# PRBonn/OverlapNet

Hardware: NVIDIA H100
Metric: scan-pairs/sec (overlap+yaw) at 64x900 (higher is better)
Workload: dtype f16

## Files before the change

### overlapnet_b200/csrc/network_tc.cu

```cuda
#include "common.cuh"
#include "hopper.cuh"

#include <cuda_fp16.h>
#include <stddef.h>
#include <stdlib.h>

namespace ovn {

using namespace hopper;

constexpr int WF = 360;
constexpr int CF = 128;
constexpr int S15 = 15;
constexpr int NB = 24;
constexpr int PAIR_ROWS = NB * NB;
constexpr int K4_PITCH = CF;

struct TcState {
  Buffer<__half> w1p;
  Buffer<__half> w2p;
  Buffer<__half> w3p;
  Buffer<float> b2eff;
  Buffer<__half> wres[kMaxLegLayers];
  Buffer<__half> actp[2];
// ... 313 lines not shown
#pragma unroll
            for (int j = 0; j < 8; ++j) sto[tt][h][j] = st + ((j ^ (ib & 7)) << 4);
          }
      }
      const uint32_t wb = S.right.slot(ui);
      PIPE_WAIT(S.right.wait(ui), kErrDeltaRightConsumer);
      float acc[2][32];
#pragma unroll
      for (int j = 0; j < 8; ++j) {
        const float m0 = __half2float(__float2half_rn(-__ldg(mu_o1 + j * 8 + 2 * t)));
        const float m1 = __half2float(__float2half_rn(-__ldg(mu_o1 + j * 8 + 2 * t + 1)));
#pragma unroll
        for (int tt = 0; tt < 2; ++tt) {
          acc[tt][4 * j + 0] = m0; acc[tt][4 * j + 1] = m1;
          acc[tt][4 * j + 2] = m0; acc[tt][4 * j + 3] = m1;
        }
      }
      uint32_t Lr[2][2][4];
#pragma unroll 1
      for (int grp = 0; grp < K4_NGROUPS; ++grp, ++gi) {
        const int cc = grp / K4_CHUNK_GROUPS, dj0 = (grp - K4_CHUNK_GROUPS * cc) * K4_GROUP;
        if (dj0 == 0) {
#pragma unroll
          for (int tt = 0; tt < 2; ++tt)
#pragma unroll
            for (int h = 0; h < 2; ++h) {
              const int r = rows[tt][h] < blk.rows ? rows[tt][h] : blk.rows - 1;
              const uint4 v = *reinterpret_cast<const uint4*>(S.L + r * K4_PITCH + ((cc ^ (r & 1)) << 5) + 8 * t);
              Lr[tt][h][0] = v.x; Lr[tt][h][1] = v.y; Lr[tt][h][2] = v.z; Lr[tt][h][3] = v.w;
            }
        }
        const uint32_t s = S.w1.slot(gi);
        const uint64_t bdesc = desc_kmajor(b_base + s * (K4_GROUP * K4_BSLICE), 1024, 128, kNoSwizzle);
        const int par = (jb + dj0) & 1;
        const __half* rw = S.Rw[wb] + dj0 * K4_PITCH + 8 * t;
        const __half* rp[2] = {rw + ((cc ^ par) << 5), rw + ((cc ^ par ^ 1) << 5)};
        uint4 rv = *reinterpret_cast<const uint4*>(rp[0]);
        PIPE_WAIT(S.w1.wait(gi), kErrDeltaW1Consumer);
        uint32_t A[2][2][4];
#pragma unroll
        for (int sl = 0; sl < K4_GROUP; ++sl)
#pragma unroll
          for (int kk = 0; kk < 2; ++kk) {
            const uint32_t r0 = kk ? rv.z : rv.x, r1 = kk ? rv.w : rv.y;
#pragma unroll
            for (int tt = 0; tt < 2; ++tt) {
              A[tt][kk][0] = absdiff_h2(Lr[tt][0][2 * kk], r0);
              A[tt][kk][1] = absdiff_h2(Lr[tt][1][2 * kk], r0);
              A[tt][kk][2] = absdiff_h2(Lr[tt][0][2 * kk + 1], r1);
              A[tt][kk][3] = absdiff_h2(Lr[tt][1][2 * kk + 1], r1);
            }
            wgmma_fence();
#pragma unroll
            for (int tt = 0; tt < 2; ++tt)
              wgmma_m64n64k16_rs(acc[tt], A[tt][kk], bdesc + ((sl * K4_BSLICE + kk * 2048) >> 4));
            wgmma_commit();
            if (kk == 1 && sl + 1 < K4_GROUP) rv = *reinterpret_cast<const uint4*>(rp[(sl + 1) & 1] + (sl + 1) * K4_PITCH);
            wgmma_wait<1>();
          }
        wgmma_wait<0>();
        S.w1.release(gi);
      }
      S.right.release(ui);
      if (jb == NB - 1 || u == u_end - 1) S.left.release(pi - 1);
      if (!S.o1s.wait_free(ui)) { atomicExch(err, kErrDeltaO1Consumer); goto done; }
#pragma unroll
      for (int tt = 0; tt < 2; ++tt)
#pragma unroll
        for (int h = 0; h < 2; ++h) {
          if (rows[tt][h] >= blk.rows) continue;
#pragma unroll
          for (int j = 0; j < 8; ++j)
            *reinterpret_cast<uint32_t*>(smem_raw + sto[tt][h][j]) = pack_h2(acc[tt][4 * j + 2 * h], acc[tt][4 * j + 2 * h + 1]);
        }
      fence_proxy_async_smem();
      S.o1s.publish(ui);
    }
  }
done:
  return;
}

constexpr int TC_WG = 2;
constexpr int TC_THREADS = TC_WG * 128 + 32;
constexpr int TC_ROWS = TC_WG * 128;
constexpr uint32_t C2_TILE = 128 * 64 * 2;
constexpr int C2_RING = 3;

struct C2Smem {
  __half A[C2_RING][TC_WG][C2_TILE / 2];
  __half B[C2_RING][2][C2_TILE / 2];
  MbarRing<C2_RING> ring;
};
constexpr size_t C2_SMEM = sizeof(C2Smem) + 1024;
static_assert(C2_SMEM <= 232448, "k_conv2_wgmma shared memory");
static_assert(offsetof(C2Smem, B) % 1024 == 0 && C2_TILE % 1024 == 0, "SWIZZLE_128B tiles on 1024-byte boundaries");

__global__ void __launch_bounds__(TC_THREADS, 1)
k_conv2_wgmma(const __half* __restrict__ o1, const __half* __restrict__ W2s, const float* __restrict__ bias2,
              const float* __restrict__ mu_x3, __half* __restrict__ x3, int64_t out_pitch, int64_t M, int fault,
              int* __restrict__ err) {
  if (fault) {
    if (threadIdx.x == 0 && blockIdx.x == 0) atomicExch(err, kErrInjectedFault);
    return;
  }
  extern __shared__ __align__(128) uint8_t smem_raw[];
  C2Smem& S = *reinterpret_cast<C2Smem*>(smem_raw + ((1024 - (smem_u32(smem_raw) & 1023)) & 1023));
  const int tid = threadIdx.x, warp = tid >> 5, lane = tid & 31;
  const Share tiles = work_share((M + TC_ROWS - 1) / TC_ROWS, blockIdx.x, gridDim.x);
  if (tid == 0) {
    S.ring.init(TC_WG * 4);
    mbar_fence_init();
  }
  __syncthreads();

  if (warp == TC_WG * 4) {
    if (lane == 0) {
      uint32_t gi = 0;
      for (int64_t tile = tiles.begin; tile < tiles.end; ++tile)
        for (int di = 0; di < S15; ++di, ++gi) {
          const uint32_t s = S.ring.slot(gi);
          PIPE_WAIT(S.ring.acquire(gi, 4 * C2_TILE), kErrConv2Producer);
          for (int h = 0; h < TC_WG; ++h)
            bulk_g2s(S.A[s][h], o1 + ((size_t)(tile * TC_WG + h) * S15 + di) * (C2_TILE / 2), C2_TILE, S.ring.bar(gi));
          bulk_g2s(S.B[s], W2s + (size_t)di * C2_TILE, 2 * C2_TILE, S.ring.bar(gi));
        }
    }
  } else {
    const int wg = warp >> 2, wi = warp & 3, g = lane >> 2, t = lane & 3;
    uint32_t gi = 0;
    bool failed = false;
    for (int64_t tile = tiles.begin; tile < tiles.end; ++tile) {
      float acc[2][64];
#pragma unroll
      for (int sub = 0; sub < 2; ++sub)
#pragma unroll
        for (int e = 0; e < 64; ++e) acc[sub][e] = 0.f;
#pragma unroll 1
      for (int di = 0; di < S15; ++di, ++gi) {
        const uint32_t s = S.ring.slot(gi);
        INFLIGHT_WAIT(S.ring.wait(gi), kErrConv2Consumer);
        const uint32_t a_base = smem_u32(S.A[s][wg]), b_base = smem_u32(S.B[s][0]);
        wgmma_fence();
#pragma unroll
        for (int kk = 0; kk < 4; ++kk)
#pragma unroll
          for (int part = 0; part < 2; ++part) {
            const uint64_t bd = desc_kmajor(b_base + part * C2_TILE + kk * 32, 16, 1024, kSwizzle128B);
#pragma unroll
            for (int sub = 0; sub < 2; ++sub)
              wgmma_m64n128k16_ss(acc[sub], desc_kmajor(a_base + sub * (C2_TILE / 2) + kk * 32, 16, 1024, kSwizzle128B), bd);
          }
        wgmma_commit();
        wgmma_wait<1>();
        if (di > 0) S.ring.release(gi - 1);
      }
      wgmma_wait<0>();
      if (failed) goto done;
      S.ring.release(gi - 1);
#pragma unroll
      for (int sub = 0; sub < 2; ++sub)
#pragma unroll
        for (int h = 0; h < 2; ++h) {
          const int64_t m = tile * TC_ROWS + wg * 128 + sub * 64 + wi * 16 + g + 8 * h;
          if (m >= M) continue;
#pragma unroll
          for (int j = 0; j < 16; ++j) {
            const int n = j * 8 + 2 * t;
            const float a = fmaxf(acc[sub][4 * j + 2 * h] + __ldg(bias2 + n), 0.f) - __ldg(mu_x3 + n);
            const float b = fmaxf(acc[sub][4 * j + 2 * h + 1] + __ldg(bias2 + n + 1), 0.f) - __ldg(mu_x3 + n + 1);
            *reinterpret_cast<uint32_t*>(x3 + ((size_t)j * out_pitch + m) * 8 + 2 * t) = pack_h2(a, b);
          }
        }
    }
  }
done:
  return;
}

constexpr int C3_AROWS = TC_ROWS + 2 * NB + 2;
constexpr uint32_t C3_PLANE = C3_AROWS * 16;
constexpr uint32_t C3_SLAB = 4 * 128 * 16;
constexpr int C3_GROUP = 2;
constexpr int C3_NSTAGES = 36 / C3_GROUP;
constexpr int C3_RING = 4;

struct C3Smem {
  __half A[2][16 * C3_PLANE / 2];
  __half B[C3_RING][C3_GROUP * C3_SLAB / 2];
  MbarRing<C3_RING> w3;
  MbarRing<2> x3;
};
static_assert(sizeof(C3Smem) <= 232448, "k_conv3_wgmma shared memory");
static_assert(offsetof(C3Smem, B) % 16 == 0 && C3_PLANE % 16 == 0, "bulk-copy alignment");

__global__ void __launch_bounds__(TC_THREADS, 1)
k_conv3_wgmma(const __half* __restrict__ X3, int64_t a_pitch, const __half* __restrict__ W3p, const float* __restrict__ bias,
              int64_t M, const float* __restrict__ wd, float* __restrict__ partial, int* __restrict__ err) {
  extern __shared__ __align__(128) uint8_t smem_raw[];
  C3Smem& S = *reinterpret_cast<C3Smem*>(smem_raw);
  const int tid = threadIdx.x, warp = tid >> 5, lane = tid & 31;
  const Share tiles = work_share(2 * ((M + TC_ROWS - 1) / TC_ROWS), blockIdx.x, gridDim.x);
  if (tid == 0) {
    S.w3.init(TC_WG * 4);
    S.x3.init(TC_WG * 4);
    mbar_fence_init();
  }
  __syncthreads();

  if (warp == TC_WG * 4) {
    if (lane == 0) {
      const uint32_t nt = (uint32_t)(tiles.end - tiles.begin);
      uint32_t ai = 0, gi = 0;
      for (uint32_t ti = 0; ti < nt; ++ti) {
        const int nh = (int)((tiles.begin + ti) & 1);
        for (int st = 0; st < C3_NSTAGES; ++st, ++gi) {
          while (ai < nt && ai <= ti + 1) {
            if (ai > ti) {
              if (!S.x3.try_acquire(ai, 16 * C3_PLANE)) break;
            } else {
              PIPE_WAIT(S.x3.acquire(ai, 16 * C3_PLANE), kErrConv3X3Producer);
            }
            const int64_t r0 = ((tiles.begin + ai) >> 1) * TC_ROWS;
            for (int pl = 0; pl < 16; ++pl)
              bulk_g2s(S.A[S.x3.slot(ai)] + pl * (C3_PLANE / 2), X3 + ((size_t)pl * a_pitch + r0) * 8, C3_PLANE, S.x3.bar(ai));
            ++ai;
          }
          PIPE_WAIT(S.w3.acquire(gi, C3_GROUP * C3_SLAB), kErrConv3W3Producer);
          bulk_g2s(S.B[S.w3.slot(gi)], W3p + ((size_t)nh * 36 + st * C3_GROUP) * (C3_SLAB / 2), C3_GROUP * C3_SLAB,
                   S.w3.bar(gi));
        }
      }
    }
  } else {
    const int wg = warp >> 2, wi = warp & 3, g = lane >> 2, t = lane & 3;
    const uint32_t b_base = smem_u32(S.B[0]);
    uint32_t gi = 0;
    bool failed = false;
    for (int64_t tile = tiles.begin; tile < tiles.end; ++tile) {
      const uint32_t ti = (uint32_t)(tile - tiles.begin);
      const int nh = (int)(tile & 1);
      const int64_t r0 = (tile >> 1) * TC_ROWS;
      PIPE_WAIT(S.x3.wait(ti), kErrConv3X3Consumer);
      const uint32_t a_rows = smem_u32(S.A[S.x3.slot(ti)]) + wg * 128 * 16;
      float acc[2][64];
#pragma unroll
      for (int sub = 0; sub < 2; ++sub)
#pragma unroll
        for (int e = 0; e < 64; ++e) acc[sub][e] = 0.f;
#pragma unroll 1
      for (int st = 0; st < C3_NSTAGES; ++st, ++gi) {
        const uint32_t s = S.w3.slot(gi);
        INFLIGHT_WAIT(S.w3.wait(gi), kErrConv3W3Consumer);
        wgmma_fence();
#pragma unroll
        for (int sl = 0; sl < C3_GROUP; ++sl) {
          const int slab = st * C3_GROUP + sl, tap = slab >> 2, c32 = slab & 3;
          const uint32_t a_tap = a_rows + ((tap / 3) * NB + tap % 3) * 16;
          const uint32_t slab_addr = b_base + s * (C3_GROUP * C3_SLAB) + sl * C3_SLAB;
#pragma unroll
          for (int kk = 0; kk < 2; ++kk) {
            const int c16 = c32 * 2 + kk;
            const uint64_t bd = desc_kmajor(slab_addr + kk * 4096, 2048, 128, kNoSwizzle);
#pragma unroll
            for (int sub = 0; sub < 2; ++sub)
              wgmma_m64n128k16_ss(acc[sub], desc_kmajor(a_tap + 2 * c16 * C3_PLANE + sub * 64 * 16, C3_PLANE, 128, kNoSwizzle), bd);
          }
        }
        wgmma_commit();
        wgmma_wait<1>();
        if (st > 0) S.w3.release(gi - 1);
      }
      wgmma_wait<0>();
      if (failed) goto done;
      S.w3.release(gi - 1);
      S.x3.release(ti);
#pragma unroll
      for (int sub = 0; sub < 2; ++sub)
#pragma unroll
        for (int h = 0; h < 2; ++h) {
          const int64_t r = r0 + wg * 128 + sub * 64 + wi * 16 + g + 8 * h;
          const int rem = (int)(r % PAIR_ROWS);
          const int yy = rem / NB, xx = rem - yy * NB;
          const bool valid = (r < M) && (yy < NB - 2) && (xx < NB - 2);
          const float* wrow = wd + (size_t)(valid ? (xx * (NB - 2) + yy) : 0) * 256 + nh * 128;
          float sum = 0.f;
#pragma unroll
          for (int j = 0; j < 16; ++j) {
            const int n = j * 8 + 2 * t;
            sum = fmaf(fmaxf(acc[sub][4 * j + 2 * h] + __ldg(bias + nh * 128 + n), 0.f), __ldg(wrow + n), sum);
            sum = fmaf(fmaxf(acc[sub][4 * j + 2 * h + 1] + __ldg(bias + nh * 128 + n + 1), 0.f), __ldg(wrow + n + 1), sum);
          }
          sum += __shfl_xor_sync(0xffffffffu, sum, 1);
          sum += __shfl_xor_sync(0xffffffffu, sum, 2);
          if (t == 0 && r < M) partial[r * 2 + nh] = valid ? sum : 0.f;
        }
    }
  }
done:
  return;
}

constexpr int C6_PARTS = C6_LT * C6_RT;
constexpr int C6_WG = 2;
constexpr int C6_THREADS = C6_WG * 128 + 32;
constexpr int C6_RING = 3;
constexpr int C6_GPITCH = 132;

struct C6Smem {
  __half R[C6_R_BYTES / 2];
  __half L[C6_RING][C6_L_BYTES / 2];
  float G[C6_WG][C6_LROWS * C6_GPITCH];
  MbarRing<C6_RING> left;
  MbarRing<1> right;
};
static_assert(sizeof(C6Smem) <= 232448, "k_corr_wgmma shared memory");
static_assert(offsetof(C6Smem, L) % 16 == 0, "bulk-copy alignment");

__global__ void __launch_bounds__(C6_THREADS, 1)
k_corr_wgmma(const __half* __restrict__ Lc, const int32_t* __restrict__ l_idx, const __half* __restrict__ Rc,
             int r_per_pair, int n_pairs, float* __restrict__ corr_part, int* __restrict__ err) {
  extern __shared__ __align__(128) uint8_t smem_raw[];
  C6Smem& S = *reinterpret_cast<C6Smem*>(smem_raw);
  const int tid = threadIdx.x, warp = tid >> 5, lane = tid & 31;
  const int q = blockIdx.x % C6_RT;
  const Share share = work_share((int64_t)n_pairs * C6_LT, blockIdx.x / C6_RT, gridDim.x / C6_RT);
  const int u_begin = (int)share.begin, u_end = (int)share.end;
  if (tid == 0) {
    S.left.init(4);
    S.right.init(C6_WG * 4);
    mbar_fence_init();
  }
  __syncthreads();

  if (warp == C6_WG * 4) {
    if (lane == 0) {
      uint32_t ri = 0, ui = 0;
      int key = -1;
      for (int u = u_begin; u < u_end; ++u, ++ui) {
        const int p = u / C6_LT, a = u - p * C6_LT;
        if ((r_per_pair ? p : 0) != key) {
          key = r_per_pair ? p : 0;
          PIPE_WAIT(S.right.acquire(ri, C6_R_BYTES), kErrCorrRightProducer);
          bulk_g2s(S.R, Rc + ((size_t)key * C6_RT + q) * (C6_R_BYTES / 2), C6_R_BYTES, S.right.bar(ri));
          ++ri;
        }
        PIPE_WAIT(S.left.acquire(ui, C6_L_BYTES), kErrCorrLeftProducer);
        bulk_g2s(S.L[S.left.slot(ui)], Lc + ((size_t)(l_idx ? l_idx[p] : p) * C6_LT + a) * (C6_L_BYTES / 2), C6_L_BYTES,
                 S.left.bar(ui));
      }
    }
  } else {
    const int wg = warp >> 2, wi = warp & 3, g = lane >> 2, t = lane & 3, tw = tid & 127;
    float* Gw = S.G[wg];
    const uint32_t r_base = smem_u32(S.R);
    uint32_t ri = 0, ui = 0;
    int key = -1;
    bool failed = false;
    for (int u = u_begin; u < u_end; ++u, ++ui) {
      const int p = u / C6_LT, a = u - p * C6_LT;
      if ((r_per_pair ? p : 0) != key) {
        if (key >= 0) S.right.release(ri - 1);
        key = r_per_pair ? p : 0;
        INFLIGHT_WAIT(S.right.wait(ri), kErrCorrRightConsumer);
        ++ri;
      }
      if ((int)(ui & 1) != wg) continue;
      const uint32_t s = S.left.slot(ui);
      INFLIGHT_WAIT(S.left.wait(ui), kErrCorrLeftConsumer);
      const uint32_t l_base = smem_u32(S.L[s]);
      float acc[64];
#pragma unroll
      for (int e = 0; e < 64; ++e) acc[e] = 0.f;
      wgmma_fence();
#pragma unroll
      for (int c16 = 0; c16 < 8; ++c16) {
        const uint64_t ah = desc_kmajor(l_base + c16 * 2 * C6_LROWS * 16, C6_LROWS * 16, 128, kNoSwizzle);
        const uint64_t al = desc_kmajor(l_base + C6_L_BYTES / 2 + c16 * 2 * C6_LROWS * 16, C6_LROWS * 16, 128, kNoSwizzle);
        const uint64_t bh = desc_kmajor(r_base + c16 * 2 * C6_RROWS * 16, C6_RROWS * 16, 128, kNoSwizzle);
        const uint64_t bl = desc_kmajor(r_base + C6_R_BYTES / 2 + c16 * 2 * C6_RROWS * 16, C6_RROWS * 16, 128, kNoSwizzle);
        wgmma_m64n128k16_ss(acc, ah, bh);
        wgmma_m64n128k16_ss(acc, al, bh);
        wgmma_m64n128k16_ss(acc, ah, bl);
      }
      wgmma_commit();
      wgmma_wait<0>();
      S.left.release(ui);
      named_bar_sync(1 + wg, 128);
#pragma unroll
      for (int j = 0; j < 16; ++j) {
        float* r0 = Gw + (wi * 16 + g) * C6_GPITCH + j * 8 + 2 * t;
        *reinterpret_cast<float2*>(r0) = make_float2(acc[4 * j], acc[4 * j + 1]);
        *reinterpret_cast<float2*>(r0 + 8 * C6_GPITCH) = make_float2(acc[4 * j + 2], acc[4 * j + 3]);
      }
      named_bar_sync(1 + wg, 128);
      const int i_lim = min(C6_LROWS, WF - a * C6_LROWS), j_lim = min(C6_RROWS, WF - q * C6_RROWS);
      float* out = corr_part + ((size_t)p * C6_PARTS + a * C6_RT + q) * WF;
      for (int d = tw; d < WF; d += 128) {
        const int dd = d - (C6_RROWS - 1);
        float sum = 0.f;
        if (d < C6_LROWS + C6_RROWS - 1) {
#pragma unroll 8
          for (int ii = 0; ii < C6_LROWS; ++ii) {
            const int jj = ii - dd;
            if (ii < i_lim && jj >= 0 && jj < j_lim) sum += Gw[ii * C6_GPITCH + jj];
          }
        }
        int k = (a * C6_LROWS - q * C6_RROWS + dd - WF / 2) % WF;
        if (k < 0) k += WF;
        out[k] = sum;
      }
    }
  }
done:
  return;
}

template <int EPI>
__global__ void __launch_bounds__(MMA_THREADS)
k_leg_mma(LegArgs g) {
  const int warp = threadIdx.x >> 5, lane = threadIdx.x & 31, gq = lane >> 2, t = lane & 3;
  const int64_t px0 = (int64_t)blockIdx.y * MMA_ROWS + warp * 16;
  if (px0 >= g.M) return;
  const int nz = (g.n_valid + 63) / 64;
  const int y = blockIdx.x, z = blockIdx.z % nz, slice = blockIdx.z / nz;
  const int64_t in_base = (int64_t)(y / g.runs_per_img) * g.in_img_planes + (int64_t)(y % g.runs_per_img) * g.in_run_planes;
  const int64_t pa = px0 + gq < g.M ? px0 + gq : g.M - 1, pb = px0 + gq + 8 < g.M ? px0 + gq + 8 : g.M - 1;
  const int n_slabs = g.kh * g.kw * 3;
  const size_t plane = (size_t)g.a_pitch * 8;
  const int per_tap = g.c8in / 2, n_it = g.kh * g.kw * per_tap;
  const int it0 = n_it * slice / g.n_split, it1 = n_it * (slice + 1) / g.n_split;
  float acc[8][4] = {};
#pragma unroll 1
  for (int it = it0; it < it1;) {
    const int tap = it / per_tap, dh = tap / g.kw, dw = tap - dh * g.kw;
    const int c8_end = (tap + 1) * per_tap < it1 ? g.c8in : (it1 - tap * per_tap) * 2;
    {
      const __half* Ah = g.A + (size_t)(in_base + (int64_t)dh * 2 * g.c8in) * plane + (size_t)dw * 8 + 2 * t;
      const __half* Al = Ah + (size_t)g.c8in * plane;
      const __half* Bh = g.Bp + ((size_t)(z * n_slabs + (dh * g.kw + dw) * 3) * g.c8in * 64 + gq) * 8 + 2 * t;
      const __half* Bl = Bh + (size_t)2 * g.c8in * 64 * 8;
#pragma unroll 1
      for (int c8 = (it - tap * per_tap) * 2; c8 < c8_end; c8 += 2) {
        const size_t o0 = (size_t)c8 * plane, o1 = o0 + plane;
        const uint32_t h0 = ld_h2(Ah + o0 + pa * 8), h1 = ld_h2(Ah + o0 + pb * 8), h2 = ld_h2(Ah + o1 + pa * 8), h3 = ld_h2(Ah + o1 + pb * 8);
        const uint32_t l0 = ld_h2(Al + o0 + pa * 8), l1 = ld_h2(Al + o0 + pb * 8), l2 = ld_h2(Al + o1 + pa * 8), l3 = ld_h2(Al + o1 + pb * 8);
        const size_t bo = (size_t)c8 * 64 * 8;
#pragma unroll
        for (int j = 0; j < 8; ++j) {
          const uint32_t wh0 = ld_h2(Bh + bo + j * 64), wh1 = ld_h2(Bh + bo + 64 * 8 + j * 64);
          const uint32_t wl0 = ld_h2(Bl + bo + j * 64), wl1 = ld_h2(Bl + bo + 64 * 8 + j * 64);
          mma16816(acc[j], h0, h1, h2, h3, wh0, wh1);
          mma16816(acc[j], l0, l1, l2, l3, wh0, wh1);
          mma16816(acc[j], h0, h1, h2, h3, wl0, wl1);
        }
      }
    }
    it = tap * per_tap + c8_end / 2;
  }
#pragma unroll
  for (int h = 0; h < 2; ++h) {
    const int64_t px = px0 + gq + 8 * h;
    if (px >= g.M) continue;
#pragma unroll
    for (int j = 0; j < 8; ++j) {
      const int n = z * 64 + j * 8 + 2 * t;
      if (n >= g.n_valid) continue;
      if (EPI == 5) {
        *reinterpret_cast<float2*>(g.part + (((size_t)slice * gridDim.x + y) * g.M + px) * g.n_valid + n) =
            make_float2(acc[j][2 * h], acc[j][2 * h + 1]);
        continue;
      }
      const float pre_a = acc[j][2 * h] + __ldg(g.bias + n), pre_b = acc[j][2 * h + 1] + __ldg(g.bias + n + 1);
      const float a = fmaxf(pre_a, 0.f), b = fmaxf(pre_b, 0.f);
      if (EPI == 4) {
        if (leg_act_unstorable(pre_a) || leg_act_unstorable(pre_b)) atomicCAS(g.err, 0, kErrNonFiniteOperand);
        const __half2 hi = __floats2half2_rn(a, b);
        const float2 hf = __half22float2(hi);
        const int64_t pl = (int64_t)y * g.out_run_planes + (n >> 3);
        *reinterpret_cast<__half2*>(g.out_planes + ((size_t)pl * g.out_pitch + px) * 8 + (n & 7)) = hi;
        *reinterpret_cast<uint32_t*>(g.out_planes + ((size_t)(pl + g.out_run_planes / 2) * g.out_pitch + px) * 8 + (n & 7)) =
            pack_h2(a - hf.x, b - hf.y);
      } else {
        *reinterpret_cast<float2*>(g.out_f32 + ((size_t)y * g.M + px) * g.n_valid + n) = make_float2(a, b);
      }
    }
  }
}

template <int EPI>
__global__ void __launch_bounds__(256)
k_leg_splitk_reduce(LegArgs g, int rows) {
  const int c8n = g.n_valid / 8;
  const int64_t i = (int64_t)blockIdx.x * blockDim.x + threadIdx.x;
  if (i >= (int64_t)rows * g.M * c8n) return;
  const int c8 = (int)(i % c8n);
  const int64_t px = (i / c8n) % g.M, y = i / c8n / g.M;
  const int64_t slice_stride = (int64_t)rows * g.M * g.n_valid;
  const float* src = g.part + (y * g.M + px) * g.n_valid + c8 * 8;
  float v[8] = {};
  for (int sl = 0; sl < g.n_split; ++sl) {
    const float4 a = __ldg(reinterpret_cast<const float4*>(src + sl * slice_stride));
    const float4 b = __ldg(reinterpret_cast<const float4*>(src + sl * slice_stride + 4));
    v[0] += a.x; v[1] += a.y; v[2] += a.z; v[3] += a.w; v[4] += b.x; v[5] += b.y; v[6] += b.z; v[7] += b.w;
  }
  bool bad = false;
#pragma unroll
  for (int e = 0; e < 8; ++e) {
    v[e] += __ldg(g.bias + c8 * 8 + e);
    bad |= leg_act_unstorable(v[e]);
    v[e] = fmaxf(v[e], 0.f);
  }
  if (EPI == 4) {
    if (bad) atomicCAS(g.err, 0, kErrNonFiniteOperand);
    __half hi[8], lo[8];
#pragma unroll
    for (int e = 0; e < 8; ++e) {
      hi[e] = __float2half_rn(v[e]);
      lo[e] = __float2half_rn(v[e] - __half2float(hi[e]));
    }
    const int64_t pl = y * g.out_run_planes + c8;
    *reinterpret_cast<uint4*>(g.out_planes + ((size_t)pl * g.out_pitch + px) * 8) = *reinterpret_cast<const uint4*>(hi);
    *reinterpret_cast<uint4*>(g.out_planes + ((size_t)(pl + g.out_run_planes / 2) * g.out_pitch + px) * 8) =
        *reinterpret_cast<const uint4*>(lo);
  } else {
    float* dst = g.out_f32 + (y * g.M + px) * g.n_valid + c8 * 8;
    *reinterpret_cast<float4*>(dst) = make_float4(v[0], v[1], v[2], v[3]);
    *reinterpret_cast<float4*>(dst + 4) = make_float4(v[4], v[5], v[6], v[7]);
  }
}

__global__ void __launch_bounds__(384)
k_corr_finalize(const float* __restrict__ part, float* __restrict__ corr_out, int32_t* __restrict__ yaw,
                const int* __restrict__ err) {
  __shared__ float s_corr[WF];
  const int p = blockIdx.x;
  for (int k = threadIdx.x; k < WF; k += blockDim.x) {
    float c = 0.f;
    for (int b = 0; b < C6_PARTS; ++b) c += part[((size_t)p * C6_PARTS + b) * WF + k];
    s_corr[k] = c;
    if (corr_out) corr_out[(size_t)p * WF + k] = c;
  }
  __syncthreads();
  if (threadIdx.x == 0) {
    int best = 0;
    float bv = s_corr[0];
    for (int k = 1; k < WF; ++k)
      if (s_corr[k] > bv) { bv = s_corr[k]; best = k; }
    yaw[p] = (*err != 0) ? INT32_MIN : 180 - best;
  }
}

__global__ void __launch_bounds__(1024)
k_o1_channel_mean(const __half* __restrict__ o1, int64_t M, float* __restrict__ mu) {
  __shared__ float part[16][64];
  const int o = threadIdx.x & 63, g = threadIdx.x >> 6;
  float acc = 0.f;
  for (int64_t m = g; m < M; m += 16)
    for (int di = 0; di < S15; ++di) acc += __half2float(o1[o1_chunk_offset(m, di, o >> 3) + (o & 7)]);
  part[g][o] = acc;
  __syncthreads();
  if (g == 0) {
    float t = 0.f;
    for (int k = 0; k < 16; ++k) t += part[k][o];
    mu[o] = __half2float(__float2half_rn(t / (float)(M * S15)));
  }
}

__global__ void __launch_bounds__(1024)
k_x3_channel_mean(const __half* __restrict__ x3, int64_t pitch, int64_t M, float* __restrict__ mu) {
  __shared__ float part[8][128];
  const int n = threadIdx.x & 127, g = threadIdx.x >> 7;
  float acc = 0.f;
  for (int64_t m = g; m < M; m += 8) acc += __half2float(x3[((size_t)(n >> 3) * pitch + m) * 8 + (n & 7)]);
  part[g][n] = acc;
  __syncthreads();
  if (g == 0) {
    float t = 0.f;
    for (int k = 0; k < 8; ++k) t += part[k][n];
    mu[n] = t / (float)M;
  }
}

__global__ void __launch_bounds__(128)
k_fold_bias2(const float* __restrict__ b2base, const float* __restrict__ mu_o1, const float* __restrict__ W2,
             float* __restrict__ b2eff) {
  const int n = threadIdx.x;
  float acc = b2base[n];
  for (int di = 0; di < S15; ++di)
    for (int o = 0; o < 64; ++o) acc = fmaf(mu_o1[o], W2[((size_t)di * 64 + o) * 128 + n], acc);
  b2eff[n] = acc;
}

__global__ void __launch_bounds__(256)
k_fold_bias3(const float* __restrict__ b3, const float* __restrict__ mu_x3, const float* __restrict__ W3,
             float* __restrict__ b3eff) {
  const int m = threadIdx.x;
  float acc = b3[m];
  for (int tap = 0; tap < 9; ++tap)
    for (int n = 0; n < 128; ++n)
      acc = fmaf(mu_x3[n], W3[((size_t)tap * 128 + n) * 256 + m], acc);
  b3eff[m] = acc;
}

__global__ void __launch_bounds__(256)
k_dense_finalize(const float* __restrict__ partial, const float* __restrict__ bd, int rows_per_pair,
                 float* __restrict__ overlap, const int* __restrict__ err) {
  __shared__ float red[256];
  const int p = blockIdx.x;
  const float* x = partial + (size_t)p * rows_per_pair * 2;
  float acc = 0.f;
  for (int i = threadIdx.x; i < rows_per_pair * 2; i += 256) acc += x[i];
  red[threadIdx.x] = acc;
  __syncthreads();
  for (int o = 128; o > 0; o >>= 1) {
    if (threadIdx.x < o) red[threadIdx.x] += red[threadIdx.x + o];
    __syncthreads();
  }
  if (threadIdx.x == 0) overlap[p] = (*err != 0) ? __int_as_float(0x7fc00000) : 1.0f / (1.0f + expf(-(red[0] + bd[0])));
}

constexpr size_t L1_DIRECT_SMEM = 48 * 1024;
constexpr size_t L1_SMALL_SMEM = 200 * 1024;

template <bool CIN4>
__global__ void __launch_bounds__(512, CIN4 ? 0 : 2)
k_leg_layer1_direct(const float* __restrict__ x, const float* __restrict__ w, const float* __restrict__ bias,
                    int n, int H_in, int W_in, int cin, int kh, int kw, int sh, int sw, int H_out, int W_out,
                    int relu, __half* __restrict__ out, int* __restrict__ err) {
  constexpr int CO = 16;
  extern __shared__ __align__(16) float w_s[];
  const int pairs = (W_out + 1) / 2;
  int64_t idx = (int64_t)blockIdx.x * blockDim.x + threadIdx.x;
  const bool active = idx < (int64_t)n * H_out * pairs;
  if (!active) idx = 0;
  const int xo = 2 * (int)(idx % pairs);
  const int64_t r = idx / pairs;
  const int y = (int)(r % H_out);
  const int64_t img = r / H_out;
  const bool has1 = xo + 1 < W_out;
  float acc0[CO], acc1[CO];
#pragma unroll
  for (int e = 0; e < CO; ++e) acc0[e] = acc1[e] = bias[e];
  const float* base0 = x + ((img * H_in + (int64_t)y * sh) * W_in + (int64_t)xo * sw) * cin;
  const float* base1 = has1 ? base0 + (int64_t)sw * cin : base0;
  for (int dh = 0; dh < kh; ++dh) {
    __syncthreads();
    for (int i = threadIdx.x; i < kw * cin * CO; i += blockDim.x) w_s[i] = w[(size_t)dh * kw * cin * CO + i];
    __syncthreads();
    for (int dw = 0; dw < kw; ++dw) {
      const int64_t off = ((int64_t)dh * W_in + dw) * cin;
      const float* pw = w_s + (size_t)(dw * cin) * CO;
      if (CIN4) {
        const float4 a = __ldg(reinterpret_cast<const float4*>(base0 + off));
        const float4 b = __ldg(reinterpret_cast<const float4*>(base1 + off));
        const float va[4] = {a.x, a.y, a.z, a.w}, vb[4] = {b.x, b.y, b.z, b.w};
#pragma unroll
        for (int c = 0; c < 4; ++c) {
#pragma unroll
          for (int q4 = 0; q4 < 4; ++q4) {
            const float4 wv = *reinterpret_cast<const float4*>(pw + c * CO + q4 * 4);
            acc0[q4 * 4 + 0] = fmaf(va[c], wv.x, acc0[q4 * 4 + 0]); acc1[q4 * 4 + 0] = fmaf(vb[c], wv.x, acc1[q4 * 4 + 0]);
            acc0[q4 * 4 + 1] = fmaf(va[c], wv.y, acc0[q4 * 4 + 1]); acc1[q4 * 4 + 1] = fmaf(vb[c], wv.y, acc1[q4 * 4 + 1]);
            acc0[q4 * 4 + 2] = fmaf(va[c], wv.z, acc0[q4 * 4 + 2]); acc1[q4 * 4 + 2] = fmaf(vb[c], wv.z, acc1[q4 * 4 + 2]);
            acc0[q4 * 4 + 3] = fmaf(va[c], wv.w, acc0[q4 * 4 + 3]); acc1[q4 * 4 + 3] = fmaf(vb[c], wv.w, acc1[q4 * 4 + 3]);
          }
        }
      } else {
        for (int c = 0; c < cin; ++c) {
          const float va = __ldg(base0 + off + c), vb = __ldg(base1 + off + c);
#pragma unroll
          for (int q4 = 0; q4 < 4; ++q4) {
            const float4 wv = *reinterpret_cast<const float4*>(pw + c * CO + q4 * 4);
            acc0[q4 * 4 + 0] = fmaf(va, wv.x, acc0[q4 * 4 + 0]); acc1[q4 * 4 + 0] = fmaf(vb, wv.x, acc1[q4 * 4 + 0]);
            acc0[q4 * 4 + 1] = fmaf(va, wv.y, acc0[q4 * 4 + 1]); acc1[q4 * 4 + 1] = fmaf(vb, wv.y, acc1[q4 * 4 + 1]);
            acc0[q4 * 4 + 2] = fmaf(va, wv.z, acc0[q4 * 4 + 2]); acc1[q4 * 4 + 2] = fmaf(vb, wv.z, acc1[q4 * 4 + 2]);
            acc0[q4 * 4 + 3] = fmaf(va, wv.w, acc0[q4 * 4 + 3]); acc1[q4 * 4 + 3] = fmaf(vb, wv.w, acc1[q4 * 4 + 3]);
          }
        }
      }
    }
  }
  if (!active) return;
#pragma unroll
  for (int p = 0; p < 2; ++p) {
    if (p == 1 && !has1) break;
    const float* acc = p ? acc1 : acc0;
#pragma unroll
    for (int g = 0; g < 2; ++g) {
      __half hi[8], lo[8];
      bool bad = false;
#pragma unroll
      for (int e = 0; e < 8; ++e) {
        const float v = relu ? fmaxf(acc[g * 8 + e], 0.f) : acc[g * 8 + e];
        bad |= leg_act_unstorable(relu ? acc[g * 8 + e] : fabsf(acc[g * 8 + e]));
        hi[e] = __float2half_rn(v);
        lo[e] = __float2half_rn(v - __half2float(hi[e]));
      }
      if (bad) atomicCAS(err, 0, kErrNonFiniteOperand);
      const int64_t plane_hi = r * 4 + g;
      *reinterpret_cast<uint4*>(out + ((size_t)plane_hi * W_out + xo + p) * 8) = *reinterpret_cast<const uint4*>(hi);
      *reinterpret_cast<uint4*>(out + ((size_t)(plane_hi + 2) * W_out + xo + p) * 8) = *reinterpret_cast<const uint4*>(lo);
    }
  }
}

template <bool CIN4>
__global__ void __launch_bounds__(256)
k_leg_layer1_small(const float* __restrict__ x, const float* __restrict__ w, const float* __restrict__ bias,
                    int n, int H_in, int W_in, int cin, int kh, int kw, int sh, int sw, int H_out, int W_out, int cout,
                    int relu, __half* __restrict__ out, int* __restrict__ err) {
  extern __shared__ __align__(16) float w_s[];
  for (int i = threadIdx.x; i < kh * kw * cin * cout; i += blockDim.x) w_s[i] = w[i];
  __syncthreads();
// ... 552 lines not shown
```

Before: 222,100.

## Stage correlation tile in the left ring slot and use three consumer warpgroups

The corr kernel drops its dedicated per-warpgroup G staging buffer and writes the wgmma accumulator into the just-consumed LEFT ring slot, using an XOR swizzle to avoid bank conflicts. The slot is released only after the diagonal reduction, with a proxy fence. The freed shared memory allows a third consumer warpgroup and a deeper 5-stage ring. The diagonal sum is rewritten so each thread walks one wrapped diagonal and splits it into two outputs, which removes the per-d loop with its branches. In exchange, slots stay occupied longer and register and shared-memory pressure change.

```diff
diff --git a/overlapnet_b200/csrc/network_tc.cu b/overlapnet_b200/csrc/network_tc.cu
--- a/overlapnet_b200/csrc/network_tc.cu
+++ b/overlapnet_b200/csrc/network_tc.cu
@@ -639,15 +639,16 @@
 }
 
 constexpr int C6_PARTS = C6_LT * C6_RT;
-constexpr int C6_WG = 2;
+constexpr int C6_WG = 3;
 constexpr int C6_THREADS = C6_WG * 128 + 32;
-constexpr int C6_RING = 3;
-constexpr int C6_GPITCH = 132;
+constexpr int C6_RING = 5;
+static_assert(C6_LROWS * C6_RROWS * 4 == C6_L_BYTES, "a staged G block fills a LEFT slot");
+
+__device__ __forceinline__ int c6_gcol(int row, int col) { return col ^ ((row & 3) << 3); }
 
 struct C6Smem {
   __half R[C6_R_BYTES / 2];
   __half L[C6_RING][C6_L_BYTES / 2];
-  float G[C6_WG][C6_LROWS * C6_GPITCH];
   MbarRing<C6_RING> left;
   MbarRing<1> right;
 };
@@ -689,7 +690,6 @@
     }
   } else {
     const int wg = warp >> 2, wi = warp & 3, g = lane >> 2, t = lane & 3, tw = tid & 127;
-    float* Gw = S.G[wg];
     const uint32_t r_base = smem_u32(S.R);
     uint32_t ri = 0, ui = 0;
     int key = -1;
@@ -702,7 +702,7 @@
         INFLIGHT_WAIT(S.right.wait(ri), kErrCorrRightConsumer);
         ++ri;
       }
-      if ((int)(ui & 1) != wg) continue;
+      if ((int)(ui % C6_WG) != wg) continue;
       const uint32_t s = S.left.slot(ui);
       INFLIGHT_WAIT(S.left.wait(ui), kErrCorrLeftConsumer);
       const uint32_t l_base = smem_u32(S.L[s]);
@@ -722,31 +722,36 @@
       }
       wgmma_commit();
       wgmma_wait<0>();
-      S.left.release(ui);
       named_bar_sync(1 + wg, 128);
+      float* Gw = reinterpret_cast<float*>(S.L[s]);
 #pragma unroll
       for (int j = 0; j < 16; ++j) {
-        float* r0 = Gw + (wi * 16 + g) * C6_GPITCH + j * 8 + 2 * t;
-        *reinterpret_cast<float2*>(r0) = make_float2(acc[4 * j], acc[4 * j + 1]);
-        *reinterpret_cast<float2*>(r0 + 8 * C6_GPITCH) = make_float2(acc[4 * j + 2], acc[4 * j + 3]);
+        const int row = wi * 16 + g, col = c6_gcol(row, j * 8 + 2 * t);
+        *reinterpret_cast<float2*>(Gw + row * C6_RROWS + col) = make_float2(acc[4 * j], acc[4 * j + 1]);
+        *reinterpret_cast<float2*>(Gw + (row + 8) * C6_RROWS + col) = make_float2(acc[4 * j + 2], acc[4 * j + 3]);
       }
       named_bar_sync(1 + wg, 128);
       const int i_lim = min(C6_LROWS, WF - a * C6_LROWS), j_lim = min(C6_RROWS, WF - q * C6_RROWS);
       float* out = corr_part + ((size_t)p * C6_PARTS + a * C6_RT + q) * WF;
-      for (int d = tw; d < WF; d += 128) {
-        const int dd = d - (C6_RROWS - 1);
-        float sum = 0.f;
-        if (d < C6_LROWS + C6_RROWS - 1) {
-#pragma unroll 8
-          for (int ii = 0; ii < C6_LROWS; ++ii) {
-            const int jj = ii - dd;
-            if (ii < i_lim && jj >= 0 && jj < j_lim) sum += Gw[ii * C6_GPITCH + jj];
-          }
-        }
-        int k = (a * C6_LROWS - q * C6_RROWS + dd - WF / 2) % WF;
+      float s1 = 0.f, s2 = 0.f;
+#pragma unroll 16
+      for (int ii = 0; ii < C6_LROWS; ++ii) {
+        const int jj = (ii + C6_RROWS - 1 - tw) & (C6_RROWS - 1);
+        const float g_ij = Gw[ii * C6_RROWS + c6_gcol(ii, jj)];
+        const float v = (ii < i_lim && jj < j_lim) ? g_ij : 0.f;
+        if (ii <= tw) s1 += v;
+        else s2 += v;
+      }
+#pragma unroll
+      for (int e = 0; e < 3; ++e) {
+        const int d = tw + 128 * e;
+        if (d >= WF) break;
+        int k = (a * C6_LROWS - q * C6_RROWS + d - (C6_RROWS - 1) - WF / 2) % WF;
         if (k < 0) k += WF;
-        out[k] = sum;
-      }
+        out[k] = e == 0 ? s1 : e == 1 ? s2 : 0.f;
+      }
+      fence_proxy_async_smem();
+      S.left.release(ui);
     }
   }
 done:
```

Result: no change. 225,300, median of 6 (+1.4%).
